# ouster-lidar/ouster-sdk

Measured on AMD Instinct MI355X. Metric: Mpoints/sec projected (decode+destagger+cartesian), 128x2048 dual-return, higher is better.
Workload: dtype u32+f64

## Files before the change

### ouster_sdk_amd/csrc/capi_cartesian.hip

```cpp
#include <new>

#include "capi_internal.h"

using namespace ouster_hip_dev;

static void host_full_lut(const ouster_hip_calib& c, std::vector<double>& direction,
                          std::vector<double>& offset) {
    const size_t w = c.w, h = c.h;
    direction.assign(w * h * 3, 0.0);
    offset.assign(w * h * 3, 0.0);
    const double* b2l = c.beam_to_lidar_transform;
    const double* tf = c.transform;
    const double bx = b2l[3], bz = b2l[11];
    double n = bx;
    if (bz != 0) n = std::sqrt(std::pow(bx, 2) + std::pow(bz, 2));
    const bool per_beam = (c.n_angles == h);
    const double step = M_PI * 2.0 / static_cast<double>(w);
    for (size_t row = 0; row < h; ++row) {
        for (size_t col = 0; col < w; ++col) {
            const size_t i = row * w + col;
            double enc, azi, alt;
            if (per_beam) {
                enc = 2.0 * M_PI - static_cast<double>(col) * step;
                azi = -c.azimuth_angles_deg[row] * M_PI / 180.0;
                alt = c.altitude_angles_deg[row] * M_PI / 180.0;
            } else {
                enc = 0;
                azi = c.azimuth_angles_deg[i] * M_PI / 180.0;
                alt = c.altitude_angles_deg[i] * M_PI / 180.0;
            }
            const double d[3] = {std::cos(enc + azi) * std::cos(alt),
                                 std::sin(enc + azi) * std::cos(alt), std::sin(alt)};
            const double o[3] = {std::cos(enc) * bx - d[0] * n, std::sin(enc) * bx - d[1] * n,
                                 -d[2] * n + bz};
            for (int r = 0; r < 3; ++r) {
                double dd = 0, oo = 0;
                for (int k = 0; k < 3; ++k) {
                    dd += d[k] * tf[r * 4 + k];
                    oo += o[k] * tf[r * 4 + k];
                }
                oo += tf[r * 4 + 3];
                direction[i * 3 + r] = dd * c.range_unit;
                offset[i * 3 + r] = oo * c.range_unit;
            }
        }
    }
}

static void host_separable_tables(const ouster_hip_calib& c, std::vector<double>& beam,
                                  std::vector<double>& col, double& n_out) {
    const size_t w = c.w, h = c.h;
    const double* b2l = c.beam_to_lidar_transform;
    const double* tf = c.transform;
    const double ru = c.range_unit;
    const double bx = b2l[3], bz = b2l[11];
    double n = bx;
    if (bz != 0) n = std::sqrt(std::pow(bx, 2) + std::pow(bz, 2));
    n_out = n;
    auto rot = [&](const double v[3], double out[3]) {
        for (int r = 0; r < 3; ++r)
            out[r] = v[0] * tf[r * 4 + 0] + v[1] * tf[r * 4 + 1] + v[2] * tf[r * 4 + 2];
    };
    beam.assign(h * 9, 0.0);
    for (size_t row = 0; row < h; ++row) {
        const double azi = -c.azimuth_angles_deg[row] * M_PI / 180.0;
        const double alt = c.altitude_angles_deg[row] * M_PI / 180.0;
        const double A = std::cos(azi) * std::cos(alt), B = std::sin(azi) * std::cos(alt),
                     Cc = std::sin(alt);
        const double u[3] = {A, B, 0}, v[3] = {-B, A, 0}, wv[3] = {0, 0, Cc};
        double ru_[3];
        rot(u, ru_);
        for (int k = 0; k < 3; ++k) beam[row * 9 + k] = ru_[k] * ru;
        rot(v, ru_);
        for (int k = 0; k < 3; ++k) beam[row * 9 + 3 + k] = ru_[k] * ru;
        rot(wv, ru_);
        for (int k = 0; k < 3; ++k) beam[row * 9 + 6 + k] = ru_[k] * ru;
    }
    col.assign(w * 5, 0.0);
    const double step = M_PI * 2.0 / static_cast<double>(w);
    for (size_t cc = 0; cc < w; ++cc) {
        const double enc = 2.0 * M_PI - static_cast<double>(cc) * step;
        const double cx = std::cos(enc), sx = std::sin(enc);
        const double o[3] = {cx * bx, sx * bx, bz};
        double ro[3];
        rot(o, ro);
        col[cc * 5 + 0] = cx;
        col[cc * 5 + 1] = sx;
        for (int k = 0; k < 3; ++k) col[cc * 5 + 2 + k] = (ro[k] + tf[k * 4 + 3]) * ru;
    }
}

static int upload(void** dptr, const void* src, size_t bytes, hipStream_t st) {
    if (counted_malloc(dptr, bytes) != hipSuccess) return -1;
    if (hipMemcpyAsync(*dptr, src, bytes, hipMemcpyHostToDevice, st) != hipSuccess) return -1;
    return hipStreamSynchronize(st) == hipSuccess ? 0 : -1;
}

extern "C" {

int ouster_hip_lut_create(ouster_hip_ctx* ctx, const ouster_hip_calib* c, ouster_hip_lut** out) {
    if (!ctx || !c || !out) return fail(OUSTER_HIP_ERR_INVALID_ARGUMENT, "NULL argument");
    if (c->w == 0 || c->h == 0)
        return fail(OUSTER_HIP_ERR_INVALID_ARGUMENT, "lut dimensions must be greater than zero");
    const size_t hw = (size_t)c->w * c->h;
    if ((c->n_angles != c->h && c->n_angles != hw) || !c->azimuth_angles_deg ||
        !c->altitude_angles_deg)
        return fail(OUSTER_HIP_ERR_INVALID_ARGUMENT, "unexpected frame dimensions");
    HIP_TRY(hipSetDevice(ctx->device));
    ouster_hip_lut* L = new (std::nothrow) ouster_hip_lut();
    if (!L) return fail(OUSTER_HIP_ERR_RUNTIME, "out of memory");
    L->device = ctx->device;
    L->w = c->w;
    L->h = c->h;
    host_full_lut(*c, L->direction, L->offset);
    int rc = 0;
    if (c->n_angles == c->h) {
        std::vector<double> beam, col;
        double n;
        host_separable_tables(*c, beam, col, n);
        L->separable = true;
        rc |= upload(&L->d_beam, beam.data(), beam.size() * 8, ctx->stream);
        rc |= upload(&L->d_col, col.data(), col.size() * 8, ctx->stream);
        L->dev.beam_tab = (const double*)L->d_beam;
        L->dev.col_tab = (const double*)L->d_col;
        L->dev.n = n;
        L->dev.full_dtype = 0;
    } else {
        rc |= upload(&L->d_dir, L->direction.data(), hw * 24, ctx->stream);
        rc |= upload(&L->d_ofs, L->offset.data(), hw * 24, ctx->stream);
        L->dev.full_dir = L->d_dir;
        L->dev.full_ofs = L->d_ofs;
        L->dev.full_dtype = OUSTER_HIP_F64;
    }
    if (rc) {
        ouster_hip_lut_destroy(L);
        return fail(OUSTER_HIP_ERR_RUNTIME, "LUT upload failed");
    }
    *out = L;
    return OUSTER_HIP_OK;
}

int ouster_hip_lut_create_from_arrays(ouster_hip_ctx* ctx, const void* direction,
                                      const void* offset, uint32_t h, uint32_t w, int dtype,
                                      ouster_hip_lut** out) {
    if (!ctx || !direction || !offset || !out)
        return fail(OUSTER_HIP_ERR_INVALID_ARGUMENT, "NULL argument");
    if (w == 0 || h == 0)
        return fail(OUSTER_HIP_ERR_INVALID_ARGUMENT, "lut dimensions must be greater than zero");
    if (!float_elem(dtype))
        return fail(OUSTER_HIP_ERR_INVALID_ARGUMENT, "LUT dtype must be F32 or F64");
    HIP_TRY(hipSetDevice(ctx->device));
    const size_t hw = (size_t)w * h, es = float_elem(dtype);
    ouster_hip_lut* L = new (std::nothrow) ouster_hip_lut();
    if (!L) return fail(OUSTER_HIP_ERR_RUNTIME, "out of memory");
    L->device = ctx->device;
    L->w = w;
    L->h = h;
    L->direction.resize(hw * 3);
    L->offset.resize(hw * 3);
    for (size_t i = 0; i < hw * 3; ++i) {
        L->direction[i] = es == 4 ? (double)((const float*)direction)[i] : ((const double*)direction)[i];
        L->offset[i] = es == 4 ? (double)((const float*)offset)[i] : ((const double*)offset)[i];
    }
    int rc = upload(&L->d_dir, direction, hw * 3 * es, ctx->stream);
    rc |= upload(&L->d_ofs, offset, hw * 3 * es, ctx->stream);
    if (rc) {
        ouster_hip_lut_destroy(L);
        return fail(OUSTER_HIP_ERR_RUNTIME, "LUT upload failed");
    }
    L->dev.full_dir = L->d_dir;
    L->dev.full_ofs = L->d_ofs;
    L->dev.full_dtype = dtype;
    *out = L;
    return OUSTER_HIP_OK;
}

int ouster_hip_lut_export(const ouster_hip_lut* L, double* direction, double* offset) {
    if (!L || !direction || !offset) return fail(OUSTER_HIP_ERR_INVALID_ARGUMENT, "NULL argument");
    memcpy(direction, L->direction.data(), L->direction.size() * 8);
    memcpy(offset, L->offset.data(), L->offset.size() * 8);
    return OUSTER_HIP_OK;
}

void ouster_hip_lut_destroy(ouster_hip_lut* L) {
    if (!L) return;
    (void)hipSetDevice(L->device);
    counted_free((void*)L->d_beam);
    counted_free((void*)L->d_col);
    counted_free((void*)L->d_dir);
    counted_free((void*)L->d_ofs);
    delete L;
}

int ouster_hip_cartesian(ouster_hip_ctx* ctx, const ouster_hip_lut* lut, const uint32_t* range,
                         void* xyz, int xyz_dtype, uint32_t n_images) {
    if (!ctx || !lut) return fail(OUSTER_HIP_ERR_INVALID_ARGUMENT, "NULL argument");
    if (!float_elem(xyz_dtype))
        return fail(OUSTER_HIP_ERR_INVALID_ARGUMENT, "xyz_dtype must be F32 or F64");
    if (n_images == 0) return OUSTER_HIP_OK;
    if (!range || !xyz) return fail(OUSTER_HIP_ERR_INVALID_ARGUMENT, "NULL image pointer");
    HIP_TRY(hipSetDevice(ctx->device));
    CartesianArgs a{};
    a.lut = lut->dev;
    a.range = range;
    a.xyz = xyz;
    a.w = lut->w;
    a.h = lut->h;
    a.n_images = n_images;
    a.xyz_dtype = xyz_dtype;
    const size_t npx = (size_t)lut->w * lut->h;
    a.vec_ok = al16(range) && al16(xyz) && (npx % 4 == 0);
    const int mode = lut->separable ? (xyz_dtype == OUSTER_HIP_F32 ? 1 : 2) : 3;
    HIP_TRY(launch_cartesian(a, mode, ctx->stream));
    return OUSTER_HIP_OK;
}

int ouster_hip_cartesian_host(ouster_hip_ctx* ctx, const ouster_hip_lut* lut, const uint32_t* range, void* xyz,
                              int xyz_dtype) {
    if (!ctx || !lut) return fail(OUSTER_HIP_ERR_INVALID_ARGUMENT, "NULL argument");
    if (!float_elem(xyz_dtype))
        return fail(OUSTER_HIP_ERR_INVALID_ARGUMENT, "xyz_dtype must be F32 or F64");
    const size_t npx = (size_t)lut->w * lut->h;
    if (npx == 0) return OUSTER_HIP_OK;
    if (!range || !xyz) return fail(OUSTER_HIP_ERR_INVALID_ARGUMENT, "NULL image pointer");
    HIP_TRY(hipSetDevice(ctx->device));
    Staging st(ctx);
    const auto in = st.input(range, npx * 4), out = st.output(xyz, npx * 3 * float_elem(xyz_dtype));
    int rc = st.stage();
    if (rc != OUSTER_HIP_OK) return rc;
    rc = ouster_hip_cartesian(ctx, lut, (const uint32_t*)st.dev(in), st.dev(out), xyz_dtype, 1);
    if (rc != OUSTER_HIP_OK) return rc;
    return st.finish();
}

}
```

### ouster_sdk_amd/csrc/decode_plan.cpp

```cpp
#include "decode_plan.h"

#include <string.h>

#include <algorithm>
#include <utility>

namespace ouster_hip_dev {

const KnobDef knob_table[] = {
    {"tile", "OUSTER_HIP_TILE", &Knobs::tile},
    {"wide", "OUSTER_HIP_WIDE", &Knobs::wide},
    {"wide_kb", "OUSTER_HIP_WIDE_KB", &Knobs::wide_kb},
    {"wide_rows", "OUSTER_HIP_WIDE_ROWS", &Knobs::wide_rows},
    {"wide_min_blocks", "OUSTER_HIP_WIDE_MIN_BLOCKS", &Knobs::wide_min_blocks},
    {"tune", "OUSTER_HIP_TUNE", &Knobs::tune},
    {"xcd", "OUSTER_HIP_XCD", &Knobs::xcd},
    {"fast", "OUSTER_HIP_FAST", &Knobs::fast},
    {"dewarp_single_pass", "OUSTER_HIP_DWF_SINGLE", &Knobs::dewarp_single_pass},
    {"beam_lds", "OUSTER_HIP_BEAM_LDS", &Knobs::beam_lds},
    {"fixup", nullptr, &Knobs::fixup},
    {"small", "OUSTER_HIP_SMALL", &Knobs::small},
    {"fixup_rows", "OUSTER_HIP_FIXUP_ROWS", &Knobs::fixup_rows},
    {"hdr_words", "OUSTER_HIP_HDR_WORDS", &Knobs::hdr_words},
    {"fixup_wide", "OUSTER_HIP_FIXUP_WIDE", &Knobs::fixup_wide},
    {"stream", "OUSTER_HIP_STREAM", &Knobs::stream},
    {"stream_rows", "OUSTER_HIP_STREAM_ROWS", &Knobs::stream_rows},
    {"stream_wait", "OUSTER_HIP_STREAM_WAIT", &Knobs::stream_wait},
    {"stream_min_tiles", "OUSTER_HIP_STREAM_MIN_TILES", &Knobs::stream_min_tiles},
    {"stream_order", "OUSTER_HIP_STREAM_ORDER", &Knobs::stream_order},
    {"slotmap", "OUSTER_HIP_SLOTMAP", &Knobs::slotmap},
    {"dwf_stream", "OUSTER_HIP_DWF_STREAM", &Knobs::dwf_stream},
    {"stream_loader", "OUSTER_HIP_STREAM_LOADER", &Knobs::stream_loader},
    {"pose_direct", "OUSTER_HIP_POSE_DIRECT", &Knobs::pose_direct},
    {"tonemap_bands", "OUSTER_HIP_TONEMAP_BANDS", &Knobs::tonemap_bands},
};
const int knob_count = (int)(sizeof knob_table / sizeof knob_table[0]);

const KnobDef* find_knob(const char* name) {
    for (const KnobDef& k : knob_table)
        if (!strcmp(k.name, name)) return &k;
    return nullptr;
}

size_t decode_lds_bytes(const Geometry& g, int tile, bool general, bool beam_lds, uint32_t slots_per_frame) {
    size_t tile_bytes = ((size_t)tile * g.col_size + 16 + 15) & ~(size_t)15;
    size_t h4 = (g.pixels_per_column + 3) & ~3u;
    size_t n = tile_bytes + (size_t)tile * 8 + 32 + h4 * 4 + XYZ_SCRATCH_BYTES;
    if (beam_lds) n += ((size_t)g.pixels_per_column * 9 + (g.pixels_per_column & 1)) * 8;
    if (general) {
        const uint32_t npo = g.columns_per_frame / g.columns_per_packet;
        n = std::max(n, slotmap_lds_bytes(g.columns_per_frame, g.columns_per_packet, slots_per_frame ? slots_per_frame : npo));
        n = (n + 15) & ~(size_t)15;
    }
    return n;
}

size_t decode_wide_lds_bytes(int tw, uint32_t rows_per_tile, uint32_t img_words) {
    return ((size_t)img_words + 3 * (size_t)tw + 4 + ((rows_per_tile + 3) & ~3u)) * 4 +
           ((size_t)rows_per_tile * 9 + (rows_per_tile & 1)) * 8 + XYZ_SCRATCH_BYTES;
}

size_t slotmap_lds_bytes(uint32_t W, uint32_t cpp, uint32_t slots_per_frame) {
    return resolve_lds_words(W, W / cpp, slots_per_frame, cpp) * 4;
}

namespace {

bool fast_possible(const PlanInput& in) {
    return in.kn.fast && (uint64_t)in.slots_per_frame * in.g.columns_per_packet == in.g.columns_per_frame;
}
size_t pose_bytes_per_col(const PlanInput& in) {
    return in.xyz_poses ? (size_t)12 * (in.xyzm == 1 ? 4 : 8) : 0;
}
uint32_t narrow_tiles(const PlanInput& in, int tile) { return (in.g.columns_per_frame + tile - 1) / tile; }

bool plan_field(const ouster_hip_bits& b, uint32_t* dws, uint32_t& n_dw, uint32_t max_dw, FieldPlan& fp) {
    fp.slot[0] = fp.slot[1] = fp.slot[2] = -1;
    fp.sh = (uint8_t)((b.offset & 3u) * 8u);
    if (b.mask == 0) return true;
    const uint32_t lo = (uint32_t)__builtin_ctzll(b.mask) >> 3, hi = (63u - (uint32_t)__builtin_clzll(b.mask)) >> 3;
    const uint32_t d0 = b.offset >> 2, first = (b.offset + lo) >> 2, last = (b.offset + hi) >> 2;
    for (uint32_t d = first; d <= last; ++d) {
        if (d - d0 > 2) return false;
        uint32_t k = 0;
        while (k < n_dw && dws[k] != d) ++k;
        if (k == n_dw) {
            if (n_dw == max_dw) return false;
            dws[n_dw++] = d;
        }
        fp.slot[d - d0] = (int8_t)k;
    }
    return true;
}

uint32_t rows_of(const TileShape& s) { return s.rows_per_tile; }
uint32_t rows_of(const StreamPlan& p) { return p.sa.tr; }
template <class Probe>
auto prefer_256_bytes(const PlanInput& in, Probe probe) -> std::pair<int, decltype(probe(0))> {
    auto p256 = probe(256);
    if (p256 && rows_of(*p256) * in.g.channel_data_size >= 256) return {256, p256};
    if (auto p128 = probe(128)) return {128, p128};
    return {p256 ? 256 : 0, p256};
}

}

NarrowPlan plan_narrow(const PlanInput& in) {
    const Geometry& g = in.g;
    const size_t pose_per_col = pose_bytes_per_col(in);
    auto lds = [&](int t, bool beam) { return decode_lds_bytes(g, t, true, beam, in.slots_per_frame); };
    int tile = 0;
    for (int t : {64, 32, 16})
        if (lds(t, false) + 16 + t * pose_per_col <= 80 * 1024) { tile = t; break; }
    if (!tile)
        for (int t : {64, 32, 16})
            if (lds(t, false) + 2048 + t * pose_per_col <= 160 * 1024) { tile = t; break; }
    if (!tile) return {0, 0u};
    while (tile > 16 && (size_t)in.n_frames * narrow_tiles(in, tile) < 512) tile /= 2;
    const int forced = in.kn.tile;
    if ((forced == 64 || forced == 32 || forced == 16) && lds(forced, false) + 2048 + forced * pose_per_col <= 160 * 1024) tile = forced;
    uint32_t beam_lds = 0;
    if (in.xyzm == 1 || in.xyzm == 2) {
        const size_t extra = 2048 + tile * pose_per_col;
        const size_t without = lds(tile, false) + extra, with = lds(tile, true) + extra;
        beam_lds = (in.kn.beam_lds && with <= 160 * 1024 && (160 * 1024) / with == (160 * 1024) / without) ? 1u : 0u;
    }
    return {tile, beam_lds};
}

std::optional<TileShape> plan_wide(const PlanInput& in, int want, WideKind kind) {
    const Geometry& g = in.g;
    const Knobs& kn = in.kn;
    const uint32_t W = g.columns_per_frame, H = g.pixels_per_column, chan = g.channel_data_size;
    const bool fast = fast_possible(in), for_fix = kind == WideKind::FIXUP, small = kind == WideKind::SMALL;
    const size_t resolver_lds = slotmap_lds_bytes(W, g.columns_per_packet, in.slots_per_frame);
    const bool mapped_ok = !fast && kn.slotmap && kn.tile == 0 && resolver_lds <= 160 * 1024;
    const size_t pose_per_col = pose_bytes_per_col(in);
    if (!((fast || mapped_ok || small) && (want == 64 || want == 128 || want == 256 || want == 512) && chan && chan % 4 == 0 &&
          W >= (uint32_t)want))
        return std::nullopt;
    if ((for_fix || small) && (want == 512 || want == 64 || in.gate_counts || resolver_lds > 64 * 1024)) return std::nullopt;
    if (in.xyz_poses & 15u) return std::nullopt;
    const uint32_t rpp = 1024u / (uint32_t)want;
    uint32_t budget = (uint32_t)(kn.wide_kb > 0 ? kn.wide_kb : 64) * 1024u;
    if (pose_per_col) budget = std::min<uint32_t>(budget, 72u * 1024u - (uint32_t)want * (uint32_t)pose_per_col);
    uint32_t tr_max = budget / ((uint32_t)want * chan) / rpp * rpp;
    tr_max = std::min(tr_max, 84u / rpp * rpp);
    if (tr_max < rpp) return std::nullopt;
    auto up = [&](uint32_t v) { return (v + rpp - 1) / rpp * rpp; };
    uint32_t nch = (H + tr_max - 1) / tr_max, tr = std::min(up((H + nch - 1) / nch), tr_max);
    for (uint32_t n2 = nch; n2 <= nch + 8 && n2 <= H; ++n2) {
        const uint32_t t2 = up((H + n2 - 1) / n2);
        if (t2 <= tr_max && t2 * n2 == H && t2 * 4 >= tr * 3) { nch = n2; tr = t2; break; }
    }
    const uint32_t tiles = (W + want - 1) / want;
    const size_t min_blocks = (size_t)std::max(kn.wide_min_blocks, 0);
    TileShape s{};
    if (small) {
        if ((size_t)in.n_frames * tiles * nch >= min_blocks) return std::nullopt;
        const uint32_t want_blocks = 2u * in.cus;
        const uint32_t need = (want_blocks + in.n_frames * tiles - 1) / (in.n_frames * tiles);
        tr = std::max(rpp, std::min(tr, H / std::max(need, 1u) / rpp * rpp));
    }
    if (for_fix) {
        const uint32_t rows = kn.fixup_rows > 0 ? (uint32_t)kn.fixup_rows : (16384u + (uint32_t)want * chan - 1u) / ((uint32_t)want * chan);
        s.fix_rows_small = std::max(rpp, std::min(tr, up(rows)));
        if (tiles > 32) return std::nullopt;
    }
    if (kn.wide_rows > 0) tr = std::min((uint32_t)kn.wide_rows, H);
    if (tr > 84) return std::nullopt;
    nch = (H + tr - 1) / tr;
    if (in.gate_counts && nch > OUSTER_HIP_GATE_CHUNKS) return std::nullopt;
    if (!for_fix && !small && (size_t)in.n_frames * tiles * nch < min_blocks) return std::nullopt;
    s.rows_per_tile = tr;
    s.row_chunks = nch;
    s.lds_col_slot = (tr * chan / 4 + 1) * 4;
    s.tiles_per_frame = tiles;
    size_t img_words = (size_t)want * (s.lds_col_slot >> 2) + 4;
    if (for_fix || small) img_words = std::max(img_words, (resolver_lds / 4 + 3) & ~(size_t)3);
    if (decode_wide_lds_bytes(want, tr, (uint32_t)img_words) + 16 + (size_t)want * pose_per_col > ((for_fix || small) ? 80u : 160u) * 1024)
        return std::nullopt;
    return s;
}

std::optional<StreamPlan> plan_stream(const PlanInput& in, int tw) {
    const Geometry& g = in.g;
    const Knobs& kn = in.kn;
    const uint32_t W = g.columns_per_frame, H = g.pixels_per_column, chan = g.channel_data_size, cpp = g.columns_per_packet;
    if (!(fast_possible(in) && in.spec != SPEC_GENERIC && in.xyzm != 3 && !in.xyz_poses && in.vec_ok &&
          (tw == 128 || tw == 256 || tw == 512 || tw == 1024)))
        return std::nullopt;
    if (W % (uint32_t)tw || (uint32_t)tw % cpp || (uint32_t)tw / cpp > 64 || chan == 0 || chan % 4) return std::nullopt;
    const uint32_t ct = W / (uint32_t)tw, per_xcd = std::max(in.cus / 8u, 1u);
    if (ct > per_xcd) return std::nullopt;
    const uint64_t frame_bytes = (uint64_t)in.slots_per_frame * in.packet_stride;
    if ((in.packets & 15) || (frame_bytes & 15)) return std::nullopt;
    const uint64_t last_end = (uint64_t)(in.slots_per_frame - 1) * in.packet_stride + g.packet_header_size +
                              (uint64_t)(cpp - 1) * g.col_size + g.col_header_size + (uint64_t)H * chan;
    if (last_end + 16 > frame_bytes) return std::nullopt;
    const uint32_t rpp = 2048u / (uint32_t)tw;
    StreamPlan p{};
    StreamArgs& sa = p.sa;
    if (!plan_field(g.col_measurement_id, sa.hdr_dw, sa.n_hdr, 8, sa.mid) ||
        !plan_field(g.col_status, sa.hdr_dw, sa.n_hdr, 8, sa.st) ||
        !plan_field(g.col_timestamp, sa.hdr_dw, sa.n_hdr, 8, sa.ts) ||
        !plan_field(g.alert_flags, sa.pkt_dw, sa.n_pkt, 4, sa.alert))
        return std::nullopt;
    auto fits = [&](uint32_t tr) -> bool {
        if (tr == 0 || tr % rpp || H % tr || (tr * chan) % 16) return false;
        sa.tr = tr;
        sa.nch = H / tr;
        sa.ncell = tr * chan / 16 + 1;
        sa.npix_instr = ((uint32_t)tw * sa.ncell + 63) / 64;
        if (sa.npix_instr > 72) return false;
        uint32_t o = sa.npix_instr * 1024u;
        sa.hdr_off = o; o += sa.n_hdr * (uint32_t)tw * 4u;
        sa.pkt_off = o; o += 6u * 256u;
        sa.off_off = o; o += ((tr + 63) / 64) * 256u;
        sa.beam_off = o; o += ((tr * 18u + 63) / 64) * 256u;
        sa.ctx_bytes = (o + 1023u) & ~1023u;
        sa.fixed_off = 2u * sa.ctx_bytes;
        sa.lds_bytes = sa.fixed_off + 3u * (uint32_t)tw * 4u + 32u;
        return sa.lds_bytes <= 160u * 1024u;
    };
    bool ok = false;
    if (kn.stream_rows > 0) ok = fits((uint32_t)kn.stream_rows);
    else
        for (uint32_t tr = H / rpp * rpp; tr >= rpp && !ok; tr -= rpp) ok = fits(tr);
    if (!ok) return std::nullopt;
    if (in.gate_counts && sa.nch > OUSTER_HIP_GATE_CHUNKS) return std::nullopt;
    sa.groups = per_xcd / ct;
    const uint64_t tiles = (uint64_t)in.n_frames * ct * sa.nch, wgs = 8ull * ct * sa.groups;
    if (kn.stream_min_tiles > 0 && tiles < wgs * (uint64_t)kn.stream_min_tiles) return std::nullopt;
    uint32_t streams = (uint32_t)__builtin_popcountll(in.plane_mask) + (uint32_t)__builtin_popcountll(in.destagger_mask);
    streams += (uint32_t)__builtin_popcount(in.xyz_mask & 3u) * (in.xyzm == 1 ? 3u : 6u);
    const uint32_t stores_per_wave = streams * (sa.tr / rpp);
    sa.wait0 = (kn.stream_wait == 0 && stores_per_wave >= 64) ? 0u : 1u;
    sa.order = (uint32_t)kn.stream_order;
    sa.loader = (kn.stream_loader > 0 && (tw == 128 || tw == 256) && !in.gate_counts && kn.stream_order == 0)
                    ? (uint32_t)std::min(kn.stream_loader, 4) : 0u;
    p.shape = TileShape{sa.tr, sa.nch, 0u, ct, 0u};
    return p;
}

Candidates plan_candidates(const PlanInput& in) {
    const Knobs& kn = in.kn;
    const bool fast = fast_possible(in);
    Candidates c;
    if (kn.small && kn.stream <= 0 && kn.wide < 0 && kn.tile == 0 && kn.fast && (fast || in.may_resolve)) {
        for (int tw : {256, 128})
            if (in.g.columns_per_frame >= (uint32_t)tw) {
                if (auto s = plan_wide(in, tw, WideKind::SMALL)) {
                    c.small_width = tw;
                    c.small_shape = *s;
                    c.resolved = in.may_resolve && (!fast || kn.small == 2);
                    return c;
                }
                break;
            }
    }
    if (kn.stream > 0) {
        if (plan_stream(in, kn.stream)) {
            c.forced_stream = kn.stream;
            return c;
        }
    } else if (kn.stream < 0 && kn.wide < 0 && kn.tile == 0) {
        c.stream_auto = prefer_256_bytes(in, [&](int tw) { return plan_stream(in, tw); }).first;
        if (c.stream_auto) {
            const int other = c.stream_auto == 256 ? 128 : 256;
            if (plan_stream(in, other)) c.stream_alt = other;
        }
    }
    if (kn.wide < 0 && fast && plan_wide(in, 256, WideKind::OPTIMISTIC)) {
        const int v[5] = {256, 128, 0, 1000 + c.stream_auto, 1000 + c.stream_alt};
        memcpy(c.variant, v, sizeof v);
        c.n = c.stream_auto ? (c.stream_alt ? 5 : 4) : 3;
    }
    return c;
}

uint64_t tuner_key(const PlanInput& in, const Candidates& c) {
    uint64_t key = 1469598103934665603ull;
    auto mix = [&](uint64_t v) { key = (key ^ v) * 1099511628211ull; };
    uint32_t lg = 0;
    while ((2u << lg) <= in.n_frames) ++lg;
    mix((uint64_t)in.spec); mix(in.g.columns_per_frame); mix(in.g.pixels_per_column); mix(in.g.channel_data_size); mix(lg); mix((uint64_t)in.xyzm);
    mix(in.plane_mask); mix(in.destagger_mask);
    mix((in.xyz_mask & 3u) | (in.gate_counts ? 4u : 0u) | (in.xyz_poses ? 8u : 0u));
    mix((uint64_t)c.stream_auto); mix((uint64_t)c.stream_alt);
    return key;
}

const char* kernel_name(Kernel k) {
    switch (k) {
        case Kernel::WIDE: return "k_decode_wide";
        case Kernel::WIDE_RESOLVED: return "k_decode_wide_resolved";
        case Kernel::STREAM: return "k_decode_stream";
        case Kernel::STREAM2: return "k_decode_stream2";
        default: return "k_decode";
    }
}

static TileShape narrow_fixup_shape(const PlanInput& in, int tile) {
    return TileShape{0u, in.resident_wgs, 0u, narrow_tiles(in, tile), 0u};
}

DecodePlan plan_decode(const PlanInput& in, const Candidates& c, int selected) {
    const Knobs& kn = in.kn;
    const bool fast = fast_possible(in);
    DecodePlan p;
    const NarrowPlan narrow = plan_narrow(in);
    if (!narrow.tile) return p;
    p.ok = true;
    p.narrow_tile = narrow.tile;
    p.beam_lds = narrow.beam_lds;

    auto take_wide = [&](int tw, const std::optional<TileShape>& s) {
        if (s) { p.kernel = Kernel::WIDE; p.cols = tw; p.shape = *s; }
        return s.has_value();
    };
    auto take_stream = [&](int tw) {
        const auto s = plan_stream(in, tw);
        if (s) { p.kernel = s->sa.loader ? Kernel::STREAM2 : Kernel::STREAM; p.cols = tw; p.shape = s->shape; p.sa = s->sa; }
        return s.has_value();
    };
    auto optimistic = [&](int tw) { return plan_wide(in, tw, WideKind::OPTIMISTIC); };
    if (c.small_width) {
        take_wide(c.small_width, c.small_shape);
        if (c.resolved) p.kernel = Kernel::WIDE_RESOLVED;
    } else if (c.forced_stream) {
        take_stream(c.forced_stream);
    } else if (kn.wide >= 0) {
        if (kn.wide) take_wide(kn.wide, optimistic(kn.wide));
    } else if (!fast) {
        const auto best = prefer_256_bytes(in, optimistic);
        take_wide(best.first, best.second);
    } else if (c.n) {
        const int sel = selected;
        if (!((sel >= 1000 && take_stream(sel - 1000)) || (sel > 0 && sel < 1000 && take_wide(sel, optimistic(sel)))) && sel != 0)
            take_wide(256, optimistic(256));
    }
    if (p.kernel == Kernel::DECODE) {
        p.cols = narrow.tile;
        p.shape = TileShape{0u, 0u, 0u, narrow_tiles(in, narrow.tile), 0u};
    }
    p.xcd_map = (kn.xcd && in.n_frames >= 8) ? 1u : 0u;
    p.mode = c.resolved ? MODE_RESOLVED : fast ? MODE_FAST : MODE_GENERAL;
    const size_t map_bytes = (size_t)in.n_frames * in.g.columns_per_frame * sizeof(int32_t) * 2;
    p.slotmap = p.kernel == Kernel::WIDE && !fast;
    if (p.slotmap) p.slotmap_bytes = map_bytes;

    if (fast && kn.fixup && !c.resolved) {
        p.fixup = Fixup::NARROW;
        p.fix_shape = narrow_fixup_shape(in, narrow.tile);
        if (kn.fixup_wide && kn.tile == 0) {
            auto fix = [&](int tw) { return plan_wide(in, tw, WideKind::FIXUP); };
            const auto best = kn.fixup_wide > 1 ? std::make_pair(kn.fixup_wide, fix(kn.fixup_wide)) : prefer_256_bytes(in, fix);
            if (best.second) {
                p.fixup = Fixup::WIDE;
                p.fix_cols = best.first;
                p.fix_shape = *best.second;
                p.slotmap_bytes = map_bytes;
            }
        }
        if (kn.hdr_words) p.hdr_words_bytes = (size_t)in.n_frames * in.g.columns_per_frame * sizeof(uint32_t);
        p.fast_tiles = p.shape.tiles_per_frame;
    }
    return p;
}

void demote_fixup(const PlanInput& in, DecodePlan& p) {
    if (p.fixup != Fixup::WIDE) return;
    p.fixup = Fixup::NARROW;
    p.fix_cols = 0;
    p.fix_shape = narrow_fixup_shape(in, p.narrow_tile);
    if (!p.slotmap) p.slotmap_bytes = 0;
}

}
```

### ouster_sdk_amd/csrc/decode_plan.h

```cpp
#pragma once
#include <stddef.h>
#include <stdint.h>

#include <optional>

#include "../../include/ouster_hip.h"

#ifndef OUSTER_XYZ_PERMUTE
#define OUSTER_XYZ_PERMUTE 1
#endif

#ifdef __HIPCC__
#define OUSTER_HOST_DEVICE __host__ __device__
#else
#define OUSTER_HOST_DEVICE
#endif

namespace ouster_hip_dev {

enum SpecId { SPEC_GENERIC = 0, SPEC_DUAL_LB, SPEC_LB, SPEC_SINGLE, SPEC_DUAL, SPEC_LEGACY };

struct Geometry {
    uint32_t pixels_per_column, columns_per_packet, columns_per_frame;
    uint32_t packet_header_size, col_header_size, channel_data_size, col_footer_size,
        packet_footer_size, col_size, lidar_packet_size;
    ouster_hip_bits col_timestamp, col_measurement_id, col_status;
    ouster_hip_bits frame_id, alert_flags, thermal_shutdown, shot_limiting,
        countdown_thermal_shutdown, countdown_shot_limiting;
};

enum DecodeMode : uint32_t {
    MODE_FAST = 0,
    MODE_FIXUP = 1,
    MODE_GENERAL = 2,
    MODE_RESOLVED = 3,
};

constexpr uint32_t FS_SEQ = 0, FS_TAG = 1, FS_TICKET = 2, FS_ANY = 20, FS_WORDS = 32;

constexpr size_t XYZ_SCRATCH_BYTES = OUSTER_XYZ_PERMUTE ? 0 : 4 * 192 * 16;

struct FieldPlan {
    int8_t slot[3];
    uint8_t sh;
};
struct StreamArgs {
    uint32_t tr, nch;
    uint32_t ncell;
    uint32_t npix_instr;
    uint32_t hdr_off, pkt_off, off_off, beam_off, ctx_bytes;
    uint32_t fixed_off;
    uint32_t n_hdr, n_pkt;
    uint32_t hdr_dw[8];
    uint32_t pkt_dw[4];
    FieldPlan mid, st, ts, alert;
    uint32_t groups;
    uint32_t wait0;
    uint32_t lds_bytes;
    uint32_t order;
    uint32_t loader;
};

OUSTER_HOST_DEVICE inline size_t resolve_lds_words(uint32_t W, uint32_t npo, uint32_t slots_per_frame, uint32_t cpp) {
    return (size_t)3 * W + npo + 2 * (size_t)slots_per_frame + (size_t)slots_per_frame * cpp + 4;
}
size_t decode_lds_bytes(const Geometry& g, int tile, bool general, bool beam_lds, uint32_t slots_per_frame = 0);
size_t decode_wide_lds_bytes(int tw, uint32_t rows_per_tile, uint32_t img_words);
size_t slotmap_lds_bytes(uint32_t W, uint32_t cpp, uint32_t slots_per_frame);

struct Knobs {
    int tile = 0, wide = -1, wide_kb = 64, wide_rows = 0, wide_min_blocks = 512, tune = 1, xcd = 1, fast = 1;
    int dewarp_single_pass = 0, beam_lds = 1, fixup = 1, small = 1, fixup_rows = 0, hdr_words = 1, fixup_wide = 1;
    int stream = -1, stream_rows = 0, stream_wait = 1, stream_min_tiles = 8, stream_order = 0, slotmap = 1;
    int dwf_stream = -1, stream_loader = 4;
    int pose_direct = 0;
    int tonemap_bands = 0;
};
struct KnobDef {
    const char* name;
    const char* env;
    int Knobs::*member;
};
extern const KnobDef knob_table[];
extern const int knob_count;
const KnobDef* find_knob(const char* name);

struct PlanInput {
    Geometry g;
    Knobs kn;
    uint32_t n_frames, slots_per_frame;
    size_t packet_stride;
    uintptr_t packets, xyz_poses;
    int spec, xyzm;
    bool vec_ok;
    uint32_t n_fields;
    uint64_t plane_mask, destagger_mask;
    uint32_t xyz_mask;
    bool gate_counts;
    uint32_t cus, resident_wgs;
    bool may_resolve;
};

struct TileShape {
    uint32_t rows_per_tile, row_chunks, lds_col_slot, tiles_per_frame, fix_rows_small;
};
enum class WideKind {
    OPTIMISTIC,
    FIXUP,
    SMALL,
};
struct StreamPlan {
    StreamArgs sa;
    TileShape shape;
};

struct NarrowPlan { int tile; uint32_t beam_lds; };
NarrowPlan plan_narrow(const PlanInput& in);
std::optional<TileShape> plan_wide(const PlanInput& in, int width, WideKind kind);
std::optional<StreamPlan> plan_stream(const PlanInput& in, int width);

struct Candidates {
    int small_width = 0;
    TileShape small_shape{};
    bool resolved = false;
    int forced_stream = 0;
    int stream_auto = 0;
    int stream_alt = 0;
    int n = 0;
    int variant[5] = {0, 0, 0, 0, 0};
};
Candidates plan_candidates(const PlanInput& in);
uint64_t tuner_key(const PlanInput& in, const Candidates& c);

enum class Kernel { DECODE, WIDE, WIDE_RESOLVED, STREAM, STREAM2 };
const char* kernel_name(Kernel k);
enum class Fixup { NONE, NARROW, WIDE };

struct DecodePlan {
    bool ok = false;
    Kernel kernel = Kernel::DECODE;
    int cols = 0;
    int narrow_tile = 0;
    TileShape shape{};
    StreamArgs sa{};
    uint32_t beam_lds = 0, mode = MODE_FAST, xcd_map = 0;
    bool slotmap = false;
    Fixup fixup = Fixup::NONE;
    int fix_cols = 0;
    TileShape fix_shape{};
    uint32_t fast_tiles = 0;
    size_t hdr_words_bytes = 0;
    size_t slotmap_bytes = 0;
};
DecodePlan plan_decode(const PlanInput& in, const Candidates& c, int selected);
inline DecodePlan plan_decode(const PlanInput& in, int selected) { return plan_decode(in, plan_candidates(in), selected); }
void demote_fixup(const PlanInput& in, DecodePlan& p);

}
```

### ouster_sdk_amd/csrc/standalone_plan.cpp

```cpp
#include "standalone_plan.h"

namespace ouster_hip_dev {

const char* destagger_route_name(DestaggerRoute r) {
    switch (r) {
        case DestaggerRoute::ROWS1: return "ROWS1";
        case DestaggerRoute::ROWS2: return "ROWS2";
        case DestaggerRoute::ROWS4: return "ROWS4";
        case DestaggerRoute::LDS: return "LDS";
        case DestaggerRoute::DIRECT: return "DIRECT";
        default: return "BYTES";
    }
}

DestaggerPlan plan_destagger(size_t row_bytes, bool pointers_aligned, int rows_env, uint32_t h, uint32_t n_images) {
    DestaggerPlan p{};
    p.rows_per_wg = 1;
    p.grid_x = h;
    p.grid_y = n_images;
    const bool al = (row_bytes % 16 == 0) && pointers_aligned;
    if (al && row_bytes <= (rows_env > 0 ? DESTAGGER_ROWS_ENV_MAX : DESTAGGER_ROWS_MAX) && rows_env != 0) {
        const uint32_t rpw = rows_env > 0 ? (uint32_t)rows_env : 2u;
        const uint32_t nchunk = (uint32_t)(row_bytes >> 4), ch = (nchunk + 255) / 256;
        p.route = ch <= 1 ? DestaggerRoute::ROWS1 : ch <= 2 ? DestaggerRoute::ROWS2 : DestaggerRoute::ROWS4;
        p.rows_per_wg = rpw;
        p.lds_bytes = 2u * (uint32_t)row_bytes;
        p.grid_x = (h + rpw - 1) / rpw;
        return p;
    }
    if (!al) p.route = DestaggerRoute::BYTES;
    else if (row_bytes <= DESTAGGER_LDS_MAX) p.route = DestaggerRoute::LDS;
    else p.route = DestaggerRoute::DIRECT;
    p.lds_bytes = p.route == DestaggerRoute::LDS ? (uint32_t)row_bytes : 0u;
    return p;
}

namespace {
uint32_t tiled_rows_per_block(uint32_t tiles, uint32_t h, uint32_t n_images) {
    uint32_t rpb = h;
    while (rpb > 16 && (size_t)tiles * n_images * ((h + rpb - 1) / rpb) < STANDALONE_MIN_WGS) rpb = (rpb + 1) / 2;
    return (rpb + 15) / 16 * 16;
}

TiledPlan generic_plan(size_t items) {
    TiledPlan p{};
    size_t blocks = (items + 255) / 256;
    if (blocks > STANDALONE_GENERIC_MAX_WGS) blocks = STANDALONE_GENERIC_MAX_WGS;
    if (blocks == 0) blocks = 1;
    p.images_per_block = 1;
    p.grid_x = (uint32_t)blocks;
    p.grid_y = 1;
    return p;
}
}

TiledPlan plan_cartesian(uint32_t w, uint32_t h, uint32_t n_images, bool vec_ok, uint32_t tile_width) {
    if (!(vec_ok && w % 4 == 0)) return generic_plan(((size_t)w * h + 3) / 4 * n_images);
    TiledPlan p{};
    p.tiled = true;
    p.tile_width = tile_width;
    const uint32_t tiles = (w + tile_width - 1) / tile_width;
    const uint32_t rpb = tiled_rows_per_block(tiles, h, n_images);
    p.rows_per_block = rpb;
    uint32_t ipb = 1;
    const size_t per_image = (size_t)tiles * ((h + rpb - 1) / rpb);
    while (ipb < CARTESIAN_MAX_GROUP && ipb * 2 <= n_images &&
           per_image * ((n_images + ipb * 2 - 1) / (ipb * 2)) >= CARTESIAN_GROUP_MIN_WGS)
        ipb *= 2;
    p.images_per_block = ipb;
    p.grid_x = tiles * ((h + rpb - 1) / rpb);
    p.grid_y = (n_images + ipb - 1) / ipb;
    return p;
}

TiledPlan plan_dewarp(uint32_t w, uint32_t h, uint32_t n_images, bool aligned, uint32_t tile_width) {
    if (!(w % 4 == 0 && aligned)) return generic_plan((size_t)w * h * n_images);
    TiledPlan p{};
    p.tiled = true;
    p.tile_width = tile_width;
    const uint32_t tiles = (w + tile_width - 1) / tile_width;
    const uint32_t rpb = tiled_rows_per_block(tiles, h, n_images);
    p.rows_per_block = rpb;
    p.images_per_block = 1;
    p.grid_x = tiles * ((h + rpb - 1) / rpb);
    p.grid_y = n_images;
    return p;
}

}
```

### ouster_sdk_amd/csrc/standalone_plan.h

```cpp
#pragma once
#include <stddef.h>
#include <stdint.h>

namespace ouster_hip_dev {

constexpr size_t DESTAGGER_ROWS_MAX = 4u << 10;
constexpr size_t DESTAGGER_ROWS_ENV_MAX = 16u << 10;
constexpr uint32_t DESTAGGER_LDS_MAX = 64u << 10;
constexpr size_t STANDALONE_MIN_WGS = 1024;
constexpr size_t CARTESIAN_GROUP_MIN_WGS = 2048;
constexpr uint32_t CARTESIAN_MAX_GROUP = 16;
constexpr size_t STANDALONE_GENERIC_MAX_WGS = 256 * 32;

enum class DestaggerRoute {
    ROWS1,
    ROWS2,
    ROWS4,
    LDS,
    DIRECT,
    BYTES,
};
const char* destagger_route_name(DestaggerRoute r);

struct DestaggerPlan {
    DestaggerRoute route;
    uint32_t rows_per_wg;
    uint32_t lds_bytes;
    uint32_t grid_x, grid_y;
};

DestaggerPlan plan_destagger(size_t row_bytes, bool pointers_aligned, int rows_env, uint32_t h, uint32_t n_images);

struct TiledPlan {
    bool tiled;
    uint32_t tile_width;
    uint32_t rows_per_block;
    uint32_t images_per_block;
    uint32_t grid_x, grid_y;
};

TiledPlan plan_cartesian(uint32_t w, uint32_t h, uint32_t n_images, bool vec_ok, uint32_t tile_width);
TiledPlan plan_dewarp(uint32_t w, uint32_t h, uint32_t n_images, bool aligned, uint32_t tile_width);

}
```

Before: 209,200.

## Add persistent warp-specialized streaming cartesian kernel with LDS double-buffering

```diff
diff --git a/ouster_sdk_amd/csrc/capi_cartesian.hip b/ouster_sdk_amd/csrc/capi_cartesian.hip
--- a/ouster_sdk_amd/csrc/capi_cartesian.hip
+++ b/ouster_sdk_amd/csrc/capi_cartesian.hip
@@ -1,6 +1,7 @@
 #include <new>
 
 #include "capi_internal.h"
+#include "k_cartesian_stream.h"
 
 using namespace ouster_hip_dev;
 
@@ -211,6 +212,12 @@
     const size_t npx = (size_t)lut->w * lut->h;
     a.vec_ok = al16(range) && al16(xyz) && (npx % 4 == 0);
     const int mode = lut->separable ? (xyz_dtype == OUSTER_HIP_F32 ? 1 : 2) : 3;
+    const int knob = ctx->knobs.cartesian_stream;
+    const CartesianStreamPlan sp = plan_cartesian_stream(a.w, a.h, n_images, a.vec_ok != 0, lut->separable, ctx->cus, knob);
+    if (sp.use) {
+        HIP_TRY(launch_cartesian_stream(a, sp, mode, knob != 2, ctx->device, ctx->stream));
+        return OUSTER_HIP_OK;
+    }
     HIP_TRY(launch_cartesian(a, mode, ctx->stream));
     return OUSTER_HIP_OK;
 }
diff --git a/ouster_sdk_amd/csrc/decode_plan.cpp b/ouster_sdk_amd/csrc/decode_plan.cpp
--- a/ouster_sdk_amd/csrc/decode_plan.cpp
+++ b/ouster_sdk_amd/csrc/decode_plan.cpp
@@ -33,6 +33,7 @@
     {"stream_loader", "OUSTER_HIP_STREAM_LOADER", &Knobs::stream_loader},
     {"pose_direct", "OUSTER_HIP_POSE_DIRECT", &Knobs::pose_direct},
     {"tonemap_bands", "OUSTER_HIP_TONEMAP_BANDS", &Knobs::tonemap_bands},
+    {"cartesian_stream", "OUSTER_HIP_CARTESIAN_STREAM", &Knobs::cartesian_stream},
 };
 const int knob_count = (int)(sizeof knob_table / sizeof knob_table[0]);
 
diff --git a/ouster_sdk_amd/csrc/decode_plan.h b/ouster_sdk_amd/csrc/decode_plan.h
--- a/ouster_sdk_amd/csrc/decode_plan.h
+++ b/ouster_sdk_amd/csrc/decode_plan.h
@@ -75,6 +75,7 @@
     int dwf_stream = -1, stream_loader = 4;
     int pose_direct = 0;
     int tonemap_bands = 0;
+    int cartesian_stream = -1;
 };
 struct KnobDef {
     const char* name;
diff --git a/ouster_sdk_amd/csrc/k_cartesian_stream.h b/ouster_sdk_amd/csrc/k_cartesian_stream.h
--- /dev/null
+++ b/ouster_sdk_amd/csrc/k_cartesian_stream.h
@@ -0,0 +1,11 @@
+#pragma once
+#include <hip/hip_runtime.h>
+
+#include "ouster_hip_dev.h"
+#include "standalone_plan.h"
+
+namespace ouster_hip_dev {
+
+hipError_t launch_cartesian_stream(const CartesianArgs& a, const CartesianStreamPlan& p, int mode, bool nt, int device, hipStream_t st);
+
+}
diff --git a/ouster_sdk_amd/csrc/k_cartesian_stream.hip b/ouster_sdk_amd/csrc/k_cartesian_stream.hip
--- /dev/null
+++ b/ouster_sdk_amd/csrc/k_cartesian_stream.hip
@@ -0,0 +1,143 @@
+#include <hip/hip_runtime.h>
+
+#include <stdint.h>
+
+#include "k_cartesian_stream.h"
+#include "kernels_common.h"
+#include "launch_util.h"
+
+namespace ouster_hip_dev {
+
+namespace {
+
+__device__ __forceinline__ void glds16(const void* g, uint32_t lds) {
+    uint32_t keep;
+    lds = __builtin_amdgcn_readfirstlane(lds);
+    asm volatile("s_mov_b32 %0, m0\n\ts_mov_b32 m0, %2\n\ts_nop 0\n\tglobal_load_lds_dwordx4 %1, off\n\ts_mov_b32 m0, %0"
+                 : "=&s"(keep) : "v"(g), "s"(lds) : "memory");
+}
+__device__ __forceinline__ void glds4(const void* g, uint32_t lds) {
+    uint32_t keep;
+    lds = __builtin_amdgcn_readfirstlane(lds);
+    asm volatile("s_mov_b32 %0, m0\n\ts_mov_b32 m0, %2\n\ts_nop 0\n\tglobal_load_lds_dword %1, off\n\ts_mov_b32 m0, %0"
+                 : "=&s"(keep) : "v"(g), "s"(lds) : "memory");
+}
+
+struct CartStreamArgs {
+    uint32_t tr, row_chunks, groups, ctx_bytes, beam_off, scratch_off;
+};
+
+constexpr int TW = (int)CARTESIAN_STREAM_TW, NP = 512;
+
+}
+
+template <int MODE, bool NT>
+__global__ __launch_bounds__(768) void k_cartesian_stream(CartesianArgs a, CartStreamArgs sp) {
+    static_assert(MODE == 1 || MODE == 2, "separable tables only");
+    extern __shared__ __align__(16) uint32_t smem[];
+
+    const uint32_t tid = threadIdx.x, lane = tid & 63u;
+    const uint32_t wave = __builtin_amdgcn_readfirstlane(tid >> 6);
+    const uint32_t W = a.w, H = a.h, TR = sp.tr, nch = sp.row_chunks, NG = sp.groups;
+    const uint32_t CT = W / TW;
+    const uint32_t xcd = blockIdx.x & 7u, kx = blockIdx.x >> 3;
+    const uint32_t ct = kx % CT, grp = kx / CT;
+    const uint32_t c0 = ct * TW;
+    if (xcd >= a.n_images) return;
+    const uint32_t items = ((a.n_images - xcd + 7u) >> 3) * nch;
+    if (grp >= items) return;
+    const uint32_t n_mine = (items - grp + NG - 1) / NG;
+    auto item = [&](uint32_t i) { return grp + NG * i; };
+    const size_t npix = (size_t)W * H;
+
+    if (wave >= (uint32_t)(NP / 64)) {
+        const uint32_t nl = (blockDim.x - NP) >> 6, li = wave - NP / 64;
+        const uint32_t lds0 = (uint32_t)(uintptr_t)smem;
+        auto fetch = [&](uint32_t s, uint32_t b) {
+            const uint32_t m = s / nch, rc = s - m * nch, img = xcd + 8u * m, r0 = rc * TR;
+            const uint32_t rows = min(TR, H - r0);
+            const uint32_t ldsb = lds0 + b * sp.ctx_bytes;
+            const uint32_t* src = a.range + (size_t)img * npix + (size_t)r0 * W + c0 + lane * 4u;
+            for (uint32_t k = li; k < rows; k += nl) glds16(src + (size_t)k * W, ldsb + k * 1024u);
+            const uint32_t* bt = (const uint32_t*)a.lut.beam_tab + (size_t)r0 * 18u;
+            const uint32_t nb = rows * 18u;
+            for (uint32_t k = li; k * 64u < nb; k += nl) {
+                const uint32_t i = k * 64u + lane;
+                glds4(bt + (i < nb ? i : nb - 1u), ldsb + sp.beam_off + k * 256u);
+            }
+            asm volatile("s_waitcnt vmcnt(0)" ::: "memory");
+        };
+        fetch(item(0), 0);
+        for (uint32_t it = 0; it < n_mine; ++it) {
+            __syncthreads();
+            if (it + 1 < n_mine) fetch(item(it + 1), (it + 1) & 1u);
+        }
+        return;
+    }
+
+    const uint32_t q = lane;
+    double cx[4], sx[4], kc[4][3];
+#pragma unroll
+    for (int c = 0; c < 4; ++c) {
+        const double* t = a.lut.col_tab + (size_t)(c0 + 4u * q + c) * 5;
+        cx[c] = t[0]; sx[c] = t[1]; kc[c][0] = t[2]; kc[c][1] = t[3]; kc[c][2] = t[4];
+    }
+#pragma unroll
+    for (int c = 0; c < 4; ++c) asm volatile("" : "+v"(cx[c]), "+v"(sx[c]), "+v"(kc[c][0]), "+v"(kc[c][1]), "+v"(kc[c][2]));
+    const double n = a.lut.n;
+
+    for (uint32_t it = 0; it < n_mine; ++it) {
+        const uint32_t s = item(it);
+        const uint32_t m = s / nch, rc = s - m * nch, img = xcd + 8u * m, r0 = rc * TR;
+        const uint32_t rows = min(TR, H - r0);
+        __syncthreads();
+        const uint8_t* ctx = (const uint8_t*)smem + (it & 1u) * sp.ctx_bytes;
+        const double* s_beam = (const double*)(ctx + sp.beam_off);
+        for (uint32_t k = wave; k < rows; k += NP / 64) {
+            const uint4 t = *(const uint4*)(ctx + k * 1024u + lane * 16u);
+            const uint32_t rng[4] = {t.x, t.y, t.z, t.w};
+            const double* b = s_beam + k * 9u;
+            const double u0 = b[0], u1 = b[1], u2 = b[2], v0 = b[3], v1 = b[4], v2 = b[5], w0 = b[6], w1 = b[7], w2 = b[8];
+            double p[4][3];
+#pragma unroll
+            for (int c = 0; c < 4; ++c) {
+                const double dd[3] = {fma(cx[c], u0, fma(sx[c], v0, w0)), fma(cx[c], u1, fma(sx[c], v1, w1)),
+                                      fma(cx[c], u2, fma(sx[c], v2, w2))};
+                const double rm = (double)rng[c] - n;
+#pragma unroll
+                for (int j = 0; j < 3; ++j) p[c][j] = rng[c] ? fma(rm, dd[j], kc[c][j]) : 0.0;
+            }
+            const size_t rowpix0 = (size_t)img * npix + (size_t)(r0 + k) * W + c0;
+            if constexpr (MODE == 1) {
+                store_xyz4_permuted<TW / 4, NT>((float*)a.xyz + rowpix0 * 3, q, p);
+            } else {
+                float4* sc = (float4*)((uint8_t*)smem + sp.scratch_off) + wave * (6 * (TW / 4));
+                union { float4 f4[6]; double t[12]; } o;
+#pragma unroll
+                for (int c = 0; c < 4; ++c)
+#pragma unroll
+                    for (int j = 0; j < 3; ++j) o.t[3 * c + j] = p[c][j];
+                store_quad_coalesced<6, TW / 4>(sc, (float4*)((double*)a.xyz + rowpix0 * 3), q, o.f4);
+            }
+        }
+    }
+}
+
+template <int MODE, bool NT>
+static hipError_t launch_form(dim3 grid, dim3 block, size_t lds, int device, hipStream_t st, const CartesianArgs& a,
+                              const CartStreamArgs& sp) {
+    static LdsGrant grant;
+    return launch_with_lds(k_cartesian_stream<MODE, NT>, grid, block, lds, device, st, grant, a, sp);
+}
+
+hipError_t launch_cartesian_stream(const CartesianArgs& a, const CartesianStreamPlan& p, int mode, bool nt, int device, hipStream_t st) {
+    if (!p.use || (mode != 1 && mode != 2) || p.loaders == 0 || p.loaders > 4) return hipErrorInvalidValue;
+    const size_t lds = (size_t)p.lds_bytes + (mode == 2 ? p.scratch_bytes : 0u);
+    if (lds > 160 * 1024) return hipErrorInvalidValue;
+    const CartStreamArgs sp{p.tr, p.row_chunks, p.groups, p.ctx_bytes, p.beam_off, p.lds_bytes};
+    const dim3 grid(8u * p.tiles * p.groups), block(NP + 64u * p.loaders);
+    if (mode == 2) return launch_form<2, false>(grid, block, lds, device, st, a, sp);
+    return nt ? launch_form<1, true>(grid, block, lds, device, st, a, sp) : launch_form<1, false>(grid, block, lds, device, st, a, sp);
+}
+
+}
diff --git a/ouster_sdk_amd/csrc/standalone_plan.cpp b/ouster_sdk_amd/csrc/standalone_plan.cpp
--- a/ouster_sdk_amd/csrc/standalone_plan.cpp
+++ b/ouster_sdk_amd/csrc/standalone_plan.cpp
@@ -73,6 +73,29 @@
     return p;
 }
 
+CartesianStreamPlan plan_cartesian_stream(uint32_t w, uint32_t h, uint32_t n_images, bool vec_ok, bool separable, uint32_t cus,
+                                          int knob) {
+    CartesianStreamPlan p{};
+    if (knob == 0 || !vec_ok || !separable || w == 0 || h == 0 || n_images == 0 || w % CARTESIAN_STREAM_TW != 0) return p;
+    p.tr = CARTESIAN_STREAM_TR;
+    p.row_chunks = (h + p.tr - 1) / p.tr;
+    p.tiles = w / CARTESIAN_STREAM_TW;
+    const uint32_t per_pair = cus / (8u * p.tiles);
+    if (per_pair == 0) return p;
+    const uint32_t most = (n_images + 7u) / 8u * p.row_chunks, least = n_images / 8u * p.row_chunks;
+    p.groups = per_pair < most ? per_pair : most;
+    if (knob < 0 && (least / p.groups < CARTESIAN_STREAM_MIN_ITEMS ||
+                     ((n_images + 7u) / 8u - n_images / 8u) * CARTESIAN_STREAM_MAX_SKEW_INV > n_images / 8u))
+        return p;
+    p.loaders = CARTESIAN_STREAM_LOADERS;
+    p.beam_off = p.tr * 1024u;
+    p.ctx_bytes = p.beam_off + (p.tr * 18u + 63u) / 64u * 256u;
+    p.lds_bytes = CARTESIAN_STREAM_RING * p.ctx_bytes;
+    p.scratch_bytes = 8u * 6u * 64u * 16u;
+    p.use = true;
+    return p;
+}
+
 TiledPlan plan_dewarp(uint32_t w, uint32_t h, uint32_t n_images, bool aligned, uint32_t tile_width) {
     if (!(w % 4 == 0 && aligned)) return generic_plan((size_t)w * h * n_images);
     TiledPlan p{};
diff --git a/ouster_sdk_amd/csrc/standalone_plan.h b/ouster_sdk_amd/csrc/standalone_plan.h
--- a/ouster_sdk_amd/csrc/standalone_plan.h
+++ b/ouster_sdk_amd/csrc/standalone_plan.h
@@ -42,4 +42,24 @@
 TiledPlan plan_cartesian(uint32_t w, uint32_t h, uint32_t n_images, bool vec_ok, uint32_t tile_width);
 TiledPlan plan_dewarp(uint32_t w, uint32_t h, uint32_t n_images, bool aligned, uint32_t tile_width);
 
+constexpr uint32_t CARTESIAN_STREAM_TW = 256, CARTESIAN_STREAM_TR = 8, CARTESIAN_STREAM_RING = 2, CARTESIAN_STREAM_LOADERS = 4;
+constexpr uint32_t CARTESIAN_STREAM_MIN_ITEMS = 8;
+constexpr uint32_t CARTESIAN_STREAM_MAX_SKEW_INV = 8;
+
+struct CartesianStreamPlan {
+    bool use;
+    uint32_t tr;
+    uint32_t row_chunks;
+    uint32_t tiles;
+    uint32_t groups;
+    uint32_t loaders;
+    uint32_t ctx_bytes;
+    uint32_t beam_off;
+    uint32_t lds_bytes;
+    uint32_t scratch_bytes;
+};
+
+CartesianStreamPlan plan_cartesian_stream(uint32_t w, uint32_t h, uint32_t n_images, bool vec_ok, bool separable, uint32_t cus,
+                                          int knob);
+
 }
```

Result: slower. 181,900 (-13.0%).
